# kenziyuliu/ChineseCheckersAgent

Measured on NVIDIA B200. Metric: env_steps_per_sec, higher is better.
Workload: dtype u64

## Files before the change

chinesecheckersagent_b200/csrc/ccx_device.cuh:

```cuda
#pragma once
#include <cstdint>
#include <cuda_runtime.h>

typedef unsigned long long u64;
typedef unsigned int u32;

#define CCX_HD __host__ __device__ __forceinline__
#ifdef __CUDA_ARCH__
#define ccx_popc(x) __popc(x)
#define ccx_popcll(x) __popcll(x)
#define ccx_umulhi(a, b) __umulhi((a), (b))
#define ccx_clz(x) __clz(x)
#define ccx_clzll(x) __clzll((long long)(x))
#define ccx_ffs(x) __ffs(x)
#else
#define ccx_popc(x) __builtin_popcount(x)
#define ccx_popcll(x) __builtin_popcountll(x)
#define ccx_umulhi(a, b) ((u32)(((u64)(u32)(a) * (u64)(u32)(b)) >> 32))
#define ccx_clz(x) ((x) ? __builtin_clz(x) : 32)
#define ccx_clzll(x) ((x) ? __builtin_clzll(x) : 64)
#define ccx_ffs(x) __builtin_ffs(x)
#endif

#define CCX_VALID 0x007F7F7F7F7F7F7FULL
#define CCX_TARGET_P1 ((1ULL << 4) | (1ULL << 5) | (1ULL << 6) | (1ULL << 13) | (1ULL << 14) | (1ULL << 22))
#define CCX_TARGET_P2 ((1ULL << 32) | (1ULL << 40) | (1ULL << 41) | (1ULL << 48) | (1ULL << 49) | (1ULL << 50))
#define CCX_START_OCC1 ((1ULL << 48) | (1ULL << 40) | (1ULL << 49) | (1ULL << 32) | (1ULL << 41) | (1ULL << 50))
#define CCX_START_OCC2 ((1ULL << 6) | (1ULL << 14) | (1ULL << 5) | (1ULL << 22) | (1ULL << 13) | (1ULL << 4))
#define CCX_START_CELLS1 (48ULL | (40ULL << 8) | (49ULL << 16) | (32ULL << 24) | (41ULL << 32) | (50ULL << 40))
#define CCX_START_CELLS2 (6ULL | (14ULL << 8) | (5ULL << 16) | (22ULL << 24) | (13ULL << 32) | (4ULL << 40))
#define CCX_START_META 0x00000000FFFFFFFFULL
#define CCX_HIST_EMPTY 0xFFFFFFFFFFFFFFFFULL

template <int D> CCX_HD u64 shd(u64 x)
{
    if (D == 0) return x >> 8;
    if (D == 1) return x << 1;
    if (D == 2) return x << 9;
    if (D == 3) return x << 8;
    if (D == 4) return x >> 1;
    return x >> 9;
}

template <int D> CCX_HD u64 jump_dir(u64 F, u64 occ, u64 empty)
{
    u64 a1 = shd<D>(F);
    u64 L = shd<D>(a1 & occ) & empty;
    u64 m1 = a1 & empty;
    u64 a2 = shd<D>(m1);
    L |= shd<D>(shd<D>(a2 & occ) & empty) & empty;
    u64 m2 = a2 & empty;
    u64 a3 = shd<D>(m2);
    L |= shd<D>(shd<D>(shd<D>(a3 & occ) & empty) & empty) & empty;
    return L;
}

CCX_HD u64 jump_round(u64 F, u64 occ, u64 empty)
{
    return jump_dir<0>(F, occ, empty) | jump_dir<1>(F, occ, empty) | jump_dir<2>(F, occ, empty) |
           jump_dir<3>(F, occ, empty) | jump_dir<4>(F, occ, empty) | jump_dir<5>(F, occ, empty);
}

CCX_HD u64 neighbours(u64 o)
{
    return shd<0>(o) | shd<1>(o) | shd<2>(o) | shd<3>(o) | shd<4>(o) | shd<5>(o);
}

CCX_HD void movegen(u64 occ_all, u64 cells, u64 (&dest)[6])
{
#pragma unroll
    for (int k = 0; k < 6; k++) dest[k] = 0;
    int id = 0;
    u64 o = 1ULL << (cells & 0xFF);
    u64 occ = occ_all & ~o;
    u64 empty = ~occ & CCX_VALID;
    u64 walks = neighbours(o) & empty;
    u64 F = o, reach = 0;
    for (;;) {
        u64 nw = jump_round(F, occ, empty) & ~(reach | o);
        reach |= nw;
        F = nw;
        if (F == 0) {
            u64 d = walks | reach;
#pragma unroll
            for (int k = 0; k < 6; k++) if (id == k) dest[k] = d;
            if (++id == 6) break;
            o = 1ULL << ((cells >> (8 * id)) & 0xFF);
            occ = occ_all & ~o;
            empty = ~occ & CCX_VALID;
            walks = neighbours(o) & empty;
            F = o;
            reach = 0;
        }
    }
}

#define CCX_JT_BYTES (7 * 7 * 128)

CCX_HD uint8_t jump_line_entry(int len, int pos, int o7)
{
    int occ = o7 & ((1 << len) - 1);
    int out = 0;
    for (int dir = -1; dir <= 1; dir += 2) {
        int b = pos + dir;
        while (b >= 0 && b < len && !((occ >> b) & 1)) b += dir;
        if (b < 0 || b >= len) continue;
        int l = 2 * b - pos;
        if (l < 0 || l >= len) continue;
        bool clear = true;
        for (int q = b + dir; q != l + dir; q += dir) if ((occ >> q) & 1) clear = false;
        if (clear) out |= 1 << l;
    }
    return (uint8_t)out;
}

CCX_HD void build_jump_table(uint8_t *T, int first, int step)
{
    for (int e = first; e < CCX_JT_BYTES; e += step) {
        int len = e / 896 + 1, pos = (e / 128) % 7, o7 = e % 128;
        T[e] = pos < len ? jump_line_entry(len, pos, o7) : 0;
    }
}

CCX_HD u64 expand_cell(int i, u64 occ, const uint8_t *__restrict__ T)
{
    const int r = i >> 3, c = i & 7;
    u32 row7 = (u32)(occ >> (8 * r)) & 0x7Fu;
    u64 L = (u64)T[6 * 896 + c * 128 + row7] << (8 * r);
    u64 colx = (occ >> c) & 0x0001010101010101ULL;
    u32 col7 = (u32)((colx * 0x0000040810204081ULL) >> 42) & 0x7Fu;
    u64 colr = ((u64)T[6 * 896 + r * 128 + col7] * 0x0002040810204081ULL) & 0x0001010101010101ULL;
    L |= colr << c;
    const int k = c - r;
    const int sh = k >= 0 ? k : -8 * k;
    const int len = 7 - (k >= 0 ? k : -k);
    const int pos = k >= 0 ? r : c;
    u64 diax = (occ >> sh) & 0x0040201008040201ULL;
    u32 dia7 = (u32)((diax * 0x0001010101010101ULL) >> 48) & 0x7Fu;
    u64 diar = ((u64)T[(len - 1) * 896 + pos * 128 + dia7] * 0x0001010101010101ULL) & 0x0040201008040201ULL;
    L |= diar << sh;
    return L;
}

#define CCX_JT2_BYTES (7 * 128 * 8)

CCX_HD void build_jump_table2(uint8_t *T2, int first, int step)
{
    for (int e = first; e < CCX_JT2_BYTES; e += step) {
        int len = e / 1024 + 1, o7 = (e / 8) % 128, pos = e % 8;
        T2[e] = pos < len ? jump_line_entry(len, pos, o7) : 0;
    }
}

CCX_HD u32 cell_diag_info2(int i)
{
    const int r = i >> 3, c = i & 7, k = c - r;
    const int sh = k >= 0 ? k : -8 * k;
    const int len = 7 - (k >= 0 ? k : -k);
    const int pos = k >= 0 ? r : c;
    return (u32)(sh & 0xFF) | ((u32)(((len > 0 ? len : 1) - 1) * 1024 + (pos & 7)) << 8);
}

CCX_HD u64 expand_cell_lut2(int i, u64 occ, const uint8_t *__restrict__ T2, const u32 *__restrict__ CI2)
{
    const u32 ci = CI2[i];
    const int r = i >> 3, c = i & 7;
    u32 row7 = (u32)(occ >> (8 * r)) & 0x7Fu;
    u64 L = (u64)T2[6 * 1024 + row7 * 8 + c] << (8 * r);
    u64 colx = (occ >> c) & 0x0001010101010101ULL;
    u32 col7 = (u32)((colx * 0x0000040810204081ULL) >> 42) & 0x7Fu;
    u64 colr = ((u64)T2[6 * 1024 + col7 * 8 + r] * 0x0002040810204081ULL) & 0x0001010101010101ULL;
    L |= colr << c;
    const int sh = (int)(ci & 0xFFu);
    u64 diax = (occ >> sh) & 0x0040201008040201ULL;
    u32 dia7 = (u32)((diax * 0x0001010101010101ULL) >> 48) & 0x7Fu;
    u64 diar = ((u64)T2[(ci >> 8) + dia7 * 8] * 0x0001010101010101ULL) & 0x0040201008040201ULL;
    L |= diar << sh;
    return L;
}

#define CCX_JT3_ROW 0
#define CCX_JT3_COL (128 * 64)
#define CCX_JT3_DIA (CCX_JT3_COL + 128 * 8 * 8)
#define CCX_JT3_NLP 29
#define CCX_JT3_BYTES (CCX_JT3_DIA + 128 * CCX_JT3_NLP * 8)

CCX_HD int tri_tbit(int cell) { return ((cell & 7) << 3) | (cell >> 3); }
CCX_HD int tri_dbyte(int k) { return (k == -4 || k == 4) ? 0 : k + 4; }
CCX_HD int tri_dbit(int cell)
{
    const int r = cell >> 3, c = cell & 7, k = c - r;
    if (k < -4 || k > 4) return 3;
    return 8 * tri_dbyte(k) + (k == 4 ? 4 : 0) + (k >= 0 ? r : c);
}
CCX_HD int tri_lp(int k, int pos)
{
    const int len = 7 - (k >= 0 ? k : -k);
    if (len < 3) return 28;
    if (len == 3) return (k > 0 ? 3 : 0) + pos;
    return (len == 4 ? 6 : len == 5 ? 10 : len == 6 ? 15 : 21) + pos;
}
CCX_HD u64 tri_cell_info(int cell)
{
    const int r = cell >> 3, c = cell & 7, k = c - r;
    const int sh = k >= 0 ? k : -8 * k;
    const int sel = (k < -4 || k > 4) ? 4 : tri_dbyte(k);
    const u32 lo = (0x8880u | (u32)sel) | ((u32)(sh & 0xFF) << 16) | ((u32)(tri_lp(k, k >= 0 ? r : c) * 8) << 24);
    const u32 hi = (0x8880u | (u32)r) | ((0x8880u | (u32)c) << 16);
    return (u64)lo | ((u64)hi << 32);
}

CCX_HD void build_jump_table3(uint8_t *T3, int first, int step)
{
    for (int e = first; e < 128 * 64; e += step) {
        int o7 = e / 64, cell = e % 64;
        T3[CCX_JT3_ROW + e] = ((CCX_VALID >> cell) & 1) ? jump_line_entry(7, cell & 7, o7) : 0;
    }
    u64 *C = reinterpret_cast<u64 *>(T3 + CCX_JT3_COL);
    for (int e = first; e < 128 * 8; e += step) {
        int o7 = e / 8, pos = e % 8;
        u32 m = pos < 7 ? jump_line_entry(7, pos, o7) : 0;
        u64 out = 0;
        for (int l = 0; l < 7; l++) if ((m >> l) & 1) out |= 1ULL << (8 * l);
        C[e] = out;
    }
    u64 *D = reinterpret_cast<u64 *>(T3 + CCX_JT3_DIA);
    for (int e = first; e < 128 * CCX_JT3_NLP; e += step) {
        int o7 = e / CCX_JT3_NLP, lp = e % CCX_JT3_NLP;
        int len, pos, occ = o7;
        if (lp < 3) { len = 3; pos = lp; }
        else if (lp < 6) { len = 3; pos = lp - 3; occ = o7 >> 4; }
        else if (lp < 10) { len = 4; pos = lp - 6; }
        else if (lp < 15) { len = 5; pos = lp - 10; }
        else if (lp < 21) { len = 6; pos = lp - 15; }
        else if (lp < 28) { len = 7; pos = lp - 21; }
        else { len = 0; pos = 0; }
        u32 m = len ? jump_line_entry(len, pos, occ) : 0;
        u64 out = 0;
        for (int l = 0; l < 7; l++) if ((m >> l) & 1) out |= 1ULL << (9 * l);
        D[e] = out;
    }
}

#ifdef __CUDA_ARCH__
static __device__ __forceinline__ u32 ccx_byte_of(u32 lo, u32 hi, u32 sel)
{
    u32 d;
    asm("prmt.b32 %0, %1, %2, %3;" : "=r"(d) : "r"(lo), "r"(hi), "r"(sel));
    return d;
}
static __device__ __forceinline__ int ccx_flo(u32 x)
{
    int d;
    asm("bfind.u32 %0, %1;" : "=r"(d) : "r"(x));
    return d;
}
#else
static inline u32 ccx_byte_of(u32 lo, u32 hi, u32 sel)
{
    const u64 v = (u64)lo | ((u64)hi << 32);
    u32 d = 0;
    for (int q = 0; q < 4; q++) {
        const u32 n = (sel >> (4 * q)) & 0xFu, b = (u32)(v >> (8 * (n & 7u))) & 0xFFu;
        d |= (n & 8u ? (b & 0x80u ? 0xFFu : 0u) : b) << (8 * q);
    }
    return d;
}
static inline int ccx_flo(u32 x) { return x ? 31 - __builtin_clz(x) : -1; }
#endif

CCX_HD u64 expand_cell_tri(int i, u64 occ, u64 occT, u64 occD, const uint8_t *__restrict__ T3, const u64 *__restrict__ CI3)
{
    const u64 ci = CI3[i];
    const u32 clo = (u32)ci, chi = (u32)(ci >> 32);
    const int r8 = i & 0x38;
    const u32 row7 = ccx_byte_of((u32)occ, (u32)(occ >> 32), chi);
    u64 L = (u64)T3[CCX_JT3_ROW + row7 * 64 + i] << r8;
    const u32 col7 = ccx_byte_of((u32)occT, (u32)(occT >> 32), chi >> 16);
    L |= *reinterpret_cast<const u64 *>(T3 + CCX_JT3_COL + col7 * 64 + r8) << (i & 7);
    const u32 dia7 = ccx_byte_of((u32)occD, (u32)(occD >> 32), clo);
    L |= *reinterpret_cast<const u64 *>(T3 + CCX_JT3_DIA + dia7 * (CCX_JT3_NLP * 8) + (clo >> 24)) << ((clo >> 16) & 0xFFu);
    return L;
}

CCX_HD void movegen_rays(u64 occ_all, u64 cells, u64 (&dest)[6], const uint8_t *__restrict__ T)
{
#pragma unroll
    for (int k = 0; k < 6; k++) dest[k] = 0;
    int id = 0;
    u64 o = 1ULL << (cells & 0xFF);
    u64 occ = occ_all & ~o;
    u64 todo = o, reach = 0;
    for (;;) {
#ifdef __CUDA_ARCH__
        int i = 63 - __clzll((long long)todo);
#else
        int i = 63 - __builtin_clzll(todo);
#endif
        todo ^= 1ULL << i;
        u64 nw = expand_cell(i, occ, T) & ~(reach | o);
        reach |= nw;
        todo |= nw;
        if (todo == 0) {
            u64 d = (neighbours(o) & ~occ & CCX_VALID) | reach;
#pragma unroll
            for (int k = 0; k < 6; k++) if (id == k) dest[k] = d;
            if (++id == 6) break;
            o = 1ULL << ((cells >> (8 * id)) & 0xFF);
            occ = occ_all & ~o;
            todo = o;
            reach = 0;
        }
    }
}

CCX_HD int select64(u64 m, u32 k)
{
    u32 lo = (u32)m, hi = (u32)(m >> 32);
    u32 c = ccx_popc(lo);
    u32 w = lo; int base = 0;
    if (k >= c) { w = hi; base = 32; k -= c; }
    c = ccx_popc(w & 0xFFFFu); if (k >= c) { w >>= 16; base += 16; k -= c; }
    c = ccx_popc(w & 0xFFu);   if (k >= c) { w >>= 8;  base += 8;  k -= c; }
    c = ccx_popc(w & 0xFu);    if (k >= c) { w >>= 4;  base += 4;  k -= c; }
    c = ccx_popc(w & 0x3u);    if (k >= c) { w >>= 2;  base += 2;  k -= c; }
    c = w & 1u;              if (k >= c) { base += 1; }
    return base;
}

CCX_HD int check_win(u64 occ1, u64 occ2)
{
    if ((occ1 & CCX_TARGET_P1) == CCX_TARGET_P1) return 1;
    if ((occ2 & CCX_TARGET_P2) == CCX_TARGET_P2) return 2;
    return 0;
}

struct Philox4 { u32 x, y, z, w; };
CCX_HD Philox4 philox4x32_10(u32 k0, u32 k1, u32 c0, u32 c1, u32 c2, u32 c3)
{
#pragma unroll
    for (int r = 0; r < 10; r++) {
        u32 h0 = ccx_umulhi(0xD2511F53u, c0), l0 = 0xD2511F53u * c0;
        u32 h1 = ccx_umulhi(0xCD9E8D57u, c2), l1 = 0xCD9E8D57u * c2;
        u32 n0 = h1 ^ c1 ^ k0, n2 = h0 ^ c3 ^ k1;
        c0 = n0; c1 = l1; c2 = n2; c3 = l0;
        k0 += 0x9E3779B9u; k1 += 0xBB67AE85u;
    }
    Philox4 o = {c0, c1, c2, c3};
    return o;
}

struct Game {
    u64 occ_me, occ_op, cells_me, cells_op, meta;
};

CCX_HD void apply_move(Game &g, int id, int from, int to)
{
    g.occ_me ^= (1ULL << from) | (1ULL << to);
    g.cells_me = (g.cells_me & ~(0xFFULL << (8 * id))) | ((u64)to << (8 * id));
    u64 meta = g.meta;
    u64 ply = ((meta >> 32) + 1) & 0xFFFF;
    g.meta = (meta & 0xFFFF000000000000ULL) ^ (1ULL << 48) | (ply << 32) | ((meta & 0xFFFF) << 16) |
             (u64)from | ((u64)to << 8);
    u64 t;
    t = g.occ_me; g.occ_me = g.occ_op; g.occ_op = t;
    t = g.cells_me; g.cells_me = g.cells_op; g.cells_op = t;
}

CCX_HD void push_hist(u64 &lo, u64 &hi, int to)
{
    hi = (hi << 8) | (lo >> 56);
    lo = (lo << 8) | (u64)to;
}

CCX_HD int level_of(int cell) { return (cell >> 3) - (cell & 7) + 6; }

CCX_HD int winner_of(const Game &g)
{
    bool p2 = (g.meta >> 48) & 1;
    return check_win(p2 ? g.occ_op : g.occ_me, p2 ? g.occ_me : g.occ_op);
}

CCX_HD void reset_start(Game &g)
{
    g.occ_me = CCX_START_OCC1; g.occ_op = CCX_START_OCC2;
    g.cells_me = CCX_START_CELLS1; g.cells_op = CCX_START_CELLS2;
    g.meta = CCX_START_META;
}

CCX_HD int pick_random(const Game &g, const u64 (&dest)[6], u32 nonempty, u32 r0, u32 r1, int &from, int &to)
{
    int j = (int)ccx_umulhi(r0, nonempty);
    int id = 0, rank = 0; u64 m = 0;
#pragma unroll
    for (int k = 0; k < 6; k++) {
        bool ne = dest[k] != 0;
        if (ne && rank == j) { id = k; m = dest[k]; }
        rank += ne;
    }
    to = select64(m, ccx_umulhi(r1, (u32)ccx_popcll(m)));
    from = (int)((g.cells_me >> (8 * id)) & 0xFF);
    return id;
}

struct TriTables {
    const uint8_t *sT; const u64 *sNB, *sCI, *sO, *sOT, *sOD;
    const u32 *sSel;
    const u64 *sW;
};

CCX_HD void tri_build(u64 cells_a, u64 cells_b, const u64 *__restrict__ sOT, const u64 *__restrict__ sOD, u64 &occT, u64 &occD)
{
    occT = 0; occD = 0;
#pragma unroll
    for (int k = 0; k < 6; k++) {
        int a = (int)((cells_a >> (8 * k)) & 0x3F), b = (int)((cells_b >> (8 * k)) & 0x3F);
        occT |= sOT[a] | sOT[b];
        occD |= sOD[a] | sOD[b];
    }
}

CCX_HD u64 expand_cell_carry(int c, u64 occ, u64 occT, u64 occD, const u64 *__restrict__ W);
template <bool WIDE = false>
CCX_HD void movegen_tri(u64 occ_all, u64 occT_all, u64 occD_all, u64 cells, u64 (&dest)[6], const TriTables &T)
{
#pragma unroll
    for (int k = 0; k < 6; k++) dest[k] = 0;
    int id = 0, cell = (int)(cells & 0x3F);
    u64 o = T.sO[cell], occ = occ_all & ~o, occT = occT_all & ~T.sOT[cell], occD = occD_all & ~T.sOD[cell];
    u64 todo = o, reach = 0;
    for (;;) {
        int c = 63 - ccx_clzll(todo);
        todo ^= T.sO[c];
        u64 nw = (WIDE ? expand_cell_carry(c, occ, occT, occD, T.sW) : expand_cell_tri(c, occ, occT, occD, T.sT, T.sCI)) & ~(reach | o);
        reach |= nw;
        todo |= nw;
        if (todo == 0) {
            u64 d = (T.sNB[cell] & ~occ) | reach;
#pragma unroll
            for (int k = 0; k < 6; k++) if (id == k) dest[k] = d;
            if (++id == 6) break;
            cell = (int)((cells >> (8 * id)) & 0x3F);
            o = T.sO[cell]; occ = occ_all & ~o; occT = occT_all & ~T.sOT[cell]; occD = occD_all & ~T.sOD[cell];
            todo = o; reach = 0;
        }
    }
}

struct JumpFill {
    u64 o, occ, occT, occD, todo, reach;
};

CCX_HD JumpFill fill_start(int cell, u64 occ_all, u64 occT_all, u64 occD_all, const TriTables &T)
{
    JumpFill f;
    f.o = 1ULL << cell;
    f.occ = occ_all & ~f.o; f.occT = occT_all & ~T.sOT[cell]; f.occD = occD_all & ~T.sOD[cell];
    f.todo = f.o; f.reach = 0;
    return f;
}

CCX_HD void fill_step(JumpFill &f, const TriTables &T)
{
    const int c = 63 - ccx_clzll(f.todo);
    f.todo ^= 1ULL << c;
    const u64 nw = expand_cell_tri(c, f.occ, f.occT, f.occD, T.sT, T.sCI) & ~(f.reach | f.o);
    f.reach |= nw;
    f.todo |= nw;
}

CCX_HD u32 walk_movable(u64 occ_me, u64 occ_all, u64 cells_me)
{
    const u64 w = occ_me & neighbours(~occ_all & CCX_VALID);
    u32 b = 0;
#pragma unroll
    for (int k = 0; k < 6; k++) b |= (u32)((w >> ((cells_me >> (8 * k)) & 0x3F)) & 1) << k;
    return b;
}

CCX_HD int pick_first_start(const Game &g, u64 occT_all, u64 occD_all, u32 r0, const TriTables &T, int &from, JumpFill &f)
{
    const u64 occ_all = g.occ_me | g.occ_op;
    u32 movable = walk_movable(g.occ_me, occ_all, g.cells_me);
    u32 nowalk = ~movable & 0x3Fu;
    while (nowalk) {
        const int k = ccx_ffs(nowalk) - 1;
        nowalk &= nowalk - 1;
        JumpFill p = fill_start((int)((g.cells_me >> (8 * k)) & 0x3F), occ_all, occT_all, occD_all, T);
        fill_step(p, T);
        if (p.reach) movable |= 1u << k;
    }
    if (!movable) return -1;
    const int id = select64(movable, ccx_umulhi(r0, (u32)ccx_popc(movable)));
    from = (int)((g.cells_me >> (8 * id)) & 0x3F);
    f = fill_start(from, occ_all, occT_all, occD_all, T);
    return id;
}

CCX_HD int pick_first_to(u64 occ_all, int from, const JumpFill &f, u32 r1, const TriTables &T)
{
    const u64 m = (T.sNB[from] & ~occ_all) | f.reach;
    return select64(m, ccx_umulhi(r1, (u32)ccx_popcll(m)));
}

CCX_HD int pick_random_first(const Game &g, u64 occT_all, u64 occD_all, u32 r0, u32 r1, const TriTables &T, int &from, int &to)
{
    JumpFill f;
    const int id = pick_first_start(g, occT_all, occD_all, r0, T, from, f);
    if (id < 0) return -1;
    while (f.todo) fill_step(f, T);
    to = pick_first_to(g.occ_me | g.occ_op, from, f, r1, T);
    return id;
}


#define CCX_SEL7_BYTES (128 * 4)
CCX_HD u32 sel7_entry(u32 v)
{
    u32 e = 0, n = 0;
    for (u32 b = 0; b < 7; b++)
        if ((v >> b) & 1u) e |= b << (3 * n++);
    return e;
}

CCX_HD u32 sel7_rank(const u32 *__restrict__ sSel, u32 v, u32 r) { return (sSel[v] >> (3 * r)) & 7u; }

CCX_HD int select64_step(u64 m, u32 k, const u32 *__restrict__ sSel)
{
    const u32 lo = (u32)m, hi = (u32)(m >> 32), c = ccx_popc(lo);
    const bool up = k >= c;
    const u32 w = up ? hi : lo;
    k -= up ? c : 0u;
    const u32 c1 = ccx_popc(w & 0xFFu), c2 = ccx_popc(w & 0xFFFFu), c3 = ccx_popc(w & 0xFFFFFFu);
    const bool p1 = k >= c1, p2 = k >= c2, p3 = k >= c3;
    const u32 below = p2 ? (p3 ? c3 : c2) : (p1 ? c1 : 0u);
    const u32 sh = p2 ? (p3 ? 24u : 16u) : (p1 ? 8u : 0u);
    const u32 v = (w >> sh) & 0xFFu, r = k - below;
    const u32 pos = r < (u32)ccx_popc(v & 0x7Fu) ? sel7_rank(sSel, v & 0x7Fu, r) : 7u;
    return (int)((up ? 32u : 0u) + sh + pos);
}

CCX_HD u32 walk_movable_step(u64 occ_me, u64 occ_all, u64 cells_me)
{
    const u64 w = (occ_me & neighbours(~occ_all & CCX_VALID)) << 8;
    const u32 slo = (u32)cells_me + 0x05060708u, shi = (u32)(cells_me >> 32) + 0x0304u;
    u32 b = 0;
#pragma unroll
    for (u32 k = 0; k < 6; k++) b |= (u32)(w >> ccx_byte_of(slo, shi, 0x8880u | k)) & (1u << k);
    return b;
}

#define CCX_DBASE_LO 0x78503018u
#define CCX_DBASE_HI 0x305078A8u
struct CarryCell { u32 rsel, csel, dsel, lp8, sh; };
CCX_HD CarryCell carry_cell(int c)
{
    const int r = c >> 3, col = c & 7, k = col - r;
    const u32 x = (u32)k + 0x8894u;
    const u32 base8 = ccx_byte_of(CCX_DBASE_LO, CCX_DBASE_HI, 0x8894u - (u32)k);
    CarryCell q;
    q.rsel = 0x8880u | (u32)r;
    q.csel = 0x8880u | (u32)col;
    q.dsel = x & ((x - 1u) | 7u);
    q.lp8 = base8 + 8u * (u32)(r < col ? r : col);
    q.sh = (u32)(k > -8 * k ? k : -8 * k);
    return q;
}

CCX_HD u64 expand_cell_carry(int c, u64 occ, u64 occT, u64 occD, const uint8_t *__restrict__ T3)
{
    CarryCell q = carry_cell(c);
    const int r8 = c & 0x38;
    const u32 row7 = ccx_byte_of((u32)occ, (u32)(occ >> 32), q.rsel);
    u64 L = (u64)T3[CCX_JT3_ROW + row7 * 64 + c] << r8;
    const u32 col7 = ccx_byte_of((u32)occT, (u32)(occT >> 32), q.csel);
    L |= *reinterpret_cast<const u64 *>(T3 + CCX_JT3_COL + col7 * 64 + r8) << (c & 7);
    const u32 dia7 = ccx_byte_of((u32)occD, (u32)(occD >> 32), q.dsel);
#ifdef __CUDA_ARCH__
    asm("" : "+r"(q.lp8));
#endif
    L |= *reinterpret_cast<const u64 *>(T3 + CCX_JT3_DIA + dia7 * (CCX_JT3_NLP * 8) + q.lp8) << q.sh;
    return L;
}

#define CCX_JTW_ROW 0
#define CCX_JTW_COL (128 * 64)
#define CCX_JTW_DIA (2 * 128 * 64)
#define CCX_JTW_BYTES (3 * 128 * 64 * 8)
CCX_HD void build_jump_table_wide(u64 *W, const uint8_t *T3, int first, int step)
{
    for (int e = first; e < 128 * 64; e += step) {
        const int o7 = e / 64, c = e % 64, r = c >> 3, col = c & 7, k = col - r;
        const bool on = (CCX_VALID >> c) & 1, dia = on && k >= -4 && k <= 4;
        const u64 ci = tri_cell_info(c);
        W[CCX_JTW_ROW + e] = on ? (u64)T3[CCX_JT3_ROW + o7 * 64 + c] << (c & 0x38) : 0;
        W[CCX_JTW_COL + e] = on ? *reinterpret_cast<const u64 *>(T3 + CCX_JT3_COL + o7 * 64 + 8 * r) << col : 0;
        W[CCX_JTW_DIA + e] = dia ? *reinterpret_cast<const u64 *>(T3 + CCX_JT3_DIA + o7 * (CCX_JT3_NLP * 8) + ((u32)ci >> 24))
                                       << ((ci >> 16) & 0xFF) : 0;
    }
}

CCX_HD u64 expand_cell_carry(int c, u64 occ, u64 occT, u64 occD, const u64 *__restrict__ W)
{
    const CarryCell q = carry_cell(c);
    const u32 row7 = ccx_byte_of((u32)occ, (u32)(occ >> 32), q.rsel);
    const u32 col7 = ccx_byte_of((u32)occT, (u32)(occT >> 32), q.csel);
    const u32 dia7 = ccx_byte_of((u32)occD, (u32)(occD >> 32), q.dsel);
#ifdef __CUDA_ARCH__
    const u32 wc = (u32)__cvta_generic_to_shared(W) + 8u * (u32)c;
    u64 a, b, d;
    asm("ld.shared.u64 %0, [%1];" : "=l"(a) : "r"(wc + row7 * 512u));
    asm("ld.shared.u64 %0, [%1+65536];" : "=l"(b) : "r"(wc + col7 * 512u));
    asm("ld.shared.u64 %0, [%1+131072];" : "=l"(d) : "r"(wc + dia7 * 512u));
    return a | b | d;
#else
    return W[CCX_JTW_ROW + row7 * 64 + c] | W[CCX_JTW_COL + col7 * 64 + c] | W[CCX_JTW_DIA + dia7 * 64 + c];
#endif
}

template <bool WIDE>
CCX_HD auto carry_tables(const TriTables &T)
{
    if constexpr (WIDE) return T.sW; else return T.sT;
}

template <class TAB>
CCX_HD void fill_step_carry(JumpFill &f, const TAB *__restrict__ tab)
{
    const int h = ccx_flo((u32)(f.todo >> 32)) | 32, l = ccx_flo((u32)f.todo);
    const int c = h > l ? h : l;
    f.todo ^= 1ULL << c;
    const u64 nw = expand_cell_carry(c, f.occ, f.occT, f.occD, tab) & ~(f.reach | f.o);
    f.reach |= nw;
    f.todo |= nw;
}

template <bool WIDE = false>
CCX_HD JumpFill carry_fill_start(int from, u64 occ_all, u64 occT_all, u64 occD_all, const TriTables &T)
{
    JumpFill f;
    f.o = 1ULL << from;
    f.occ = occ_all & ~f.o; f.occT = occT_all & ~T.sOT[from]; f.occD = occD_all & ~T.sOD[from];
    f.todo = expand_cell_carry(from, occ_all, occT_all, occD_all, carry_tables<WIDE>(T));
    f.reach = (T.sNB[from] & ~occ_all) | f.todo;
    return f;
}

template <bool WIDE = false>
CCX_HD int carry_ply_start(const Game &g, u64 occT_all, u64 occD_all, u32 r0, const TriTables &T, int &from, JumpFill &f)
{
    const u64 occ_all = g.occ_me | g.occ_op;
    u32 movable = walk_movable_step(g.occ_me, occ_all, g.cells_me);
    u32 nowalk = ~movable & 0x3Fu;
    while (nowalk) {
        const int k = ccx_ffs(nowalk) - 1;
        nowalk &= nowalk - 1;
        if (expand_cell_carry((int)((g.cells_me >> (8 * k)) & 0x3F), occ_all, occT_all, occD_all, carry_tables<WIDE>(T)))
            movable |= 1u << k;
    }
    if (!movable) return -1;
    const int id = (int)sel7_rank(T.sSel, movable, ccx_umulhi(r0, (u32)ccx_popc(movable)));
    from = (int)ccx_byte_of((u32)g.cells_me, (u32)(g.cells_me >> 32), 0x8880u | (u32)id);
    f = carry_fill_start<WIDE>(from, occ_all, occT_all, occD_all, T);
    return id;
}

CCX_HD int carry_ply_to(const JumpFill &f, u32 r1, const TriTables &T)
{
    return select64_step(f.reach, ccx_umulhi(r1, (u32)ccx_popcll(f.reach)), T.sSel);
}

CCX_HD u64 diag_mask(int l)
{
    const u64 D0 = 0x0040201008040201ULL;
    int k = 6 - l;
    if (k >= 0) return (D0 << k) & ((1ULL << (8 * (7 - k))) - 1ULL) & CCX_VALID;
    return (D0 << (8 * (-k))) & CCX_VALID;
}

CCX_HD int greedy_candidates(const Game &g, const u64 (&dest)[6], u64 (&cand)[6])
{
    bool p2 = (g.meta >> 48) & 1;
    int dist[6], start[6];
    int max_dist = -100;
#pragma unroll
    for (int k = 0; k < 6; k++) {
        u32 levels = 0;
#pragma unroll
        for (int l = 0; l < 13; l++) {
            const u64 dm = diag_mask(l);
            levels |= (dest[k] & dm) ? (1u << l) : 0u;
        }
        start[k] = level_of((int)((g.cells_me >> (8 * k)) & 0xFF));
        int best_end = p2 ? (31 - ccx_clz(levels)) : (ccx_ffs(levels) - 1);
        dist[k] = levels ? (p2 ? best_end - start[k] : start[k] - best_end) : -100;
        max_dist = dist[k] > max_dist ? dist[k] : max_dist;
    }
    int s_star = p2 ? 100 : -100;
#pragma unroll
    for (int k = 0; k < 6; k++)
        if (dist[k] == max_dist) s_star = p2 ? (start[k] < s_star ? start[k] : s_star) : (start[k] > s_star ? start[k] : s_star);
    int total = 0;
    if (max_dist == -100) {
#pragma unroll
        for (int k = 0; k < 6; k++) cand[k] = 0;
        return 0;
    }
    u64 end_mask = diag_mask(p2 ? s_star + max_dist : s_star - max_dist);
#pragma unroll
    for (int k = 0; k < 6; k++) {
        cand[k] = (dist[k] == max_dist && start[k] == s_star) ? (dest[k] & end_mask) : 0;
        total += ccx_popcll(cand[k]);
    }
    return total;
}

CCX_HD int pick_candidate(const Game &g, const u64 (&cand)[6], int total, u32 r0, int &from, int &to)
{
    int pick = (int)ccx_umulhi(r0, (u32)total);
    int id = 0; u64 m = 0; int base = 0; bool found = false;
#pragma unroll
    for (int k = 0; k < 6; k++) {
        int c = ccx_popcll(cand[k]);
        if (!found && pick < base + c) { id = k; m = cand[k]; pick -= base; found = true; }
        base += c;
    }
    to = select64(m, (u32)pick);
    from = (int)((g.cells_me >> (8 * id)) & 0xFF);
    return id;
}

CCX_HD bool repetition_stop(u64 lo, u64 hi)
{
    u64 seen = 0;
#pragma unroll
    for (int q = 0; q < 4; q++) {
        seen |= 1ULL << ((lo >> (16 * q)) & 63);
        seen |= 1ULL << ((hi >> (16 * q)) & 63);
    }
    return ccx_popcll(seen) <= 3;
}

CCX_HD u64 undo_in_cells(u64 cells, int from, int to)
{
#pragma unroll
    for (int k = 0; k < 6; k++)
        if (((cells >> (8 * k)) & 0xFF) == (u64)to) cells = (cells & ~(0xFFULL << (8 * k))) | ((u64)from << (8 * k));
    return cells;
}
```

Measured before the change: 37.28 billion.

## Add fast path for all-movable pieces and compute walk blockers as bitmask

Result: faster. 39.43 billion (median of 6 runs) (+5.8%).

```diff
diff --git a/chinesecheckersagent_b200/csrc/ccx_device.cuh b/chinesecheckersagent_b200/csrc/ccx_device.cuh
--- a/chinesecheckersagent_b200/csrc/ccx_device.cuh
+++ b/chinesecheckersagent_b200/csrc/ccx_device.cuh
@@ -540,14 +540,10 @@
     return (int)((up ? 32u : 0u) + sh + pos);
 }
 
-CCX_HD u32 walk_movable_step(u64 occ_me, u64 occ_all, u64 cells_me)
-{
-    const u64 w = (occ_me & neighbours(~occ_all & CCX_VALID)) << 8;
-    const u32 slo = (u32)cells_me + 0x05060708u, shi = (u32)(cells_me >> 32) + 0x0304u;
-    u32 b = 0;
-#pragma unroll
-    for (u32 k = 0; k < 6; k++) b |= (u32)(w >> ccx_byte_of(slo, shi, 0x8880u | k)) & (1u << k);
-    return b;
+CCX_HD u64 nowalk_cells(u64 occ_me, u64 occ_all)
+{
+    const u64 e = ~occ_all & CCX_VALID, l = e << 1, r = e >> 1;
+    return occ_me & ~(((e | l) << 8) | l | ((e | r) >> 8) | r);
 }
 
 #define CCX_DBASE_LO 0x78503018u
@@ -559,8 +555,8 @@
     const u32 x = (u32)k + 0x8894u;
     const u32 base8 = ccx_byte_of(CCX_DBASE_LO, CCX_DBASE_HI, 0x8894u - (u32)k);
     CarryCell q;
-    q.rsel = 0x8880u | (u32)r;
-    q.csel = 0x8880u | (u32)col;
+    q.rsel = 0x8880u + (u32)r;
+    q.csel = 0x8880u + (u32)col;
     q.dsel = x & ((x - 1u) | 7u);
     q.lp8 = base8 + 8u * (u32)(r < col ? r : col);
     q.sh = (u32)(k > -8 * k ? k : -8 * k);
@@ -618,6 +614,15 @@
 #endif
 }
 
+CCX_HD u64 or_disjoint(u64 a, u64 b)
+{
+    u32 lo = (u32)a + (u32)b, hi = (u32)(a >> 32) + (u32)(b >> 32);
+#ifdef __CUDA_ARCH__
+    asm("" : "+r"(lo), "+r"(hi));
+#endif
+    return (u64)lo | ((u64)hi << 32);
+}
+
 template <bool WIDE>
 CCX_HD auto carry_tables(const TriTables &T)
 {
@@ -631,7 +636,7 @@
     const int c = h > l ? h : l;
     f.todo ^= 1ULL << c;
     const u64 nw = expand_cell_carry(c, f.occ, f.occT, f.occD, tab) & ~(f.reach | f.o);
-    f.reach |= nw;
+    f.reach = or_disjoint(f.reach, nw);
     f.todo |= nw;
 }
 
@@ -650,17 +655,27 @@
 CCX_HD int carry_ply_start(const Game &g, u64 occT_all, u64 occD_all, u32 r0, const TriTables &T, int &from, JumpFill &f)
 {
     const u64 occ_all = g.occ_me | g.occ_op;
-    u32 movable = walk_movable_step(g.occ_me, occ_all, g.cells_me);
-    u32 nowalk = ~movable & 0x3Fu;
-    while (nowalk) {
-        const int k = ccx_ffs(nowalk) - 1;
-        nowalk &= nowalk - 1;
-        if (expand_cell_carry((int)((g.cells_me >> (8 * k)) & 0x3F), occ_all, occT_all, occD_all, carry_tables<WIDE>(T)))
-            movable |= 1u << k;
-    }
+    int id = (int)ccx_umulhi(r0, 6u);
+    from = (int)ccx_byte_of((u32)g.cells_me, (u32)(g.cells_me >> 32), 0x8880u + (u32)id);
+    f = carry_fill_start<WIDE>(from, occ_all, occT_all, occD_all, T);
+    u64 nowalk = nowalk_cells(g.occ_me, occ_all);
+    if (!nowalk) return id;
+    u64 stuck = 0;
+    do {
+        const int c = 63 - ccx_clzll(nowalk);
+        nowalk ^= 1ULL << c;
+        if (!expand_cell_carry(c, occ_all, occT_all, occD_all, carry_tables<WIDE>(T))) stuck |= 1ULL << c;
+    } while (nowalk);
+    u64 cells = g.cells_me;
+#ifdef __CUDA_ARCH__
+    asm volatile("" : "+l"(cells));
+#endif
+    u32 movable = 0;
+#pragma unroll
+    for (int k = 0; k < 6; k++) movable |= (u32)(~stuck >> ((cells >> (8 * k)) & 0x3F) & 1) << k;
     if (!movable) return -1;
-    const int id = (int)sel7_rank(T.sSel, movable, ccx_umulhi(r0, (u32)ccx_popc(movable)));
-    from = (int)ccx_byte_of((u32)g.cells_me, (u32)(g.cells_me >> 32), 0x8880u | (u32)id);
+    id = (int)sel7_rank(T.sSel, movable, ccx_umulhi(r0, (u32)ccx_popc(movable)));
+    from = (int)ccx_byte_of((u32)g.cells_me, (u32)(g.cells_me >> 32), 0x8880u + (u32)id);
     f = carry_fill_start<WIDE>(from, occ_all, occT_all, occD_all, T);
     return id;
 }
```
